# Illumina/canvas

Measured on AMD Instinct MI355X. Metric: genome-bins/sec (bin+clean+partition), higher is better.
Workload: dtype u8/int32 (bin), f32/f64 (clean, viterbi); 1 GPU; BASELINE configs[2]: whole-genome GRCh38 60x single sample, full bin+clean+partition HIP path on 1 MI355X per sample; bins_after_clean=4686240, bin_size=534, partition=PerSampleHMM, clean_flags=-g -s -r --local-sd-metric-file, segments=250, samples=1

## Files before the change

### canvas_amd/csrc/hmm.hip

```cpp
#include "common.hpp"
#include <type_traits>
#include "select.hpp"
#include "quantize.hpp"
#include <mutex>
#include <cmath>
#include <thread>
#include <cstring>
#include <limits>
#include <algorithm>

#define NSTATE 5

struct HmmParams {
    double logA[NSTATE][NSTATE];
    double logPi[NSTATE];
    int32_t tableLen;
    double maxThreshold;
};

__global__ void __launch_bounds__(256) k_keys_cov_f32(const double* __restrict__ cov, int64_t n, uint32_t* __restrict__ keys) {
    int64_t i = (int64_t)blockIdx.x * 256 + threadIdx.x;
    if (i < n) keys[i] = key_of_float((float)cov[i]);
}

// ... 232 lines not shown
            e = eNext;
        }
        __syncthreads();
        if (l < steps)
            psi[C.begin + t0 + l] = (uint16_t)(sPsi[0][l] | (sPsi[1][l] << 3) | (sPsi[2][l] << 6) | (sPsi[3][l] << 9) | (sPsi[4][l] << 12));
        __syncthreads();
    }
    double d[NSTATE];
#pragma unroll
    for (int i = 0; i < NSTATE; i++) d[i] = readlane_f64(delta, i);
    if (l == 0) {
        int best = -1; double m1 = NEG;
#pragma unroll
        for (int i = 0; i < NSTATE; i++) if (d[i] > m1) { best = i; m1 = d[i]; }
        lastState[cidx] = best;
    }
}


#define VB 128
#define VW0 16
#define VW 128
#define VW2 64
#define PQ 8
#define MAP_IDENT (0u | (1u << 3) | (2u << 6) | (3u << 9) | (4u << 12))
struct VitBlock { int32_t chrom; int32_t t0; };
struct __attribute__((aligned(4))) VecI4 { int v[4]; };
struct __attribute__((aligned(8))) VecD2 { double v[2]; };
struct __attribute__((aligned(2))) VecH8 { uint32_t w[4]; };

template <int J, bool TWO = false>
__device__ __forceinline__ void vit_state(const double (&d)[NSTATE], double e, const HmmParams& P, double& outDelta, uint32_t& outArg) {
    const double NEG = -1.7976931348623157e308;
    const double cOff = e + P.logA[J == 0 ? 1 : 0][J], cDiag = e + P.logA[J][J];
    const double t_0 = d[0] + (TWO ? (J == 0 ? cDiag : cOff) : (e + P.logA[0][J]));
    const double t_1 = d[1] + (TWO ? (J == 1 ? cDiag : cOff) : (e + P.logA[1][J]));
    const double t_2 = d[2] + (TWO ? (J == 2 ? cDiag : cOff) : (e + P.logA[2][J]));
    const double t_3 = d[3] + (TWO ? (J == 3 ? cDiag : cOff) : (e + P.logA[3][J]));
    const double t_4 = d[4] + (TWO ? (J == 4 ? cDiag : cOff) : (e + P.logA[4][J]));
    double a = __builtin_fmax(__builtin_fmax(__builtin_fmax(t_0, t_1), __builtin_fmax(t_2, t_3)), t_4);
    uint32_t ia = t_3 == a ? 3u : 4u;
    ia = t_2 == a ? 2u : ia; ia = t_1 == a ? 1u : ia; ia = t_0 == a ? 0u : ia;
    if (!(a > NEG)) { a = NEG; ia = 0; }
    outDelta = a; outArg = ia;
}
template <bool TWO = false>
__device__ __forceinline__ uint32_t vit_step5(double (&d)[NSTATE], const double (&e)[NSTATE], const HmmParams& P) {
    double n0, n1, n2, n3, n4; uint32_t a0, a1, a2, a3, a4;
    vit_state<0, TWO>(d, e[0], P, n0, a0); vit_state<1, TWO>(d, e[1], P, n1, a1); vit_state<2, TWO>(d, e[2], P, n2, a2);
    vit_state<3, TWO>(d, e[3], P, n3, a3); vit_state<4, TWO>(d, e[4], P, n4, a4);
    d[0] = n0; d[1] = n1; d[2] = n2; d[3] = n3; d[4] = n4;
    return a0 | (a1 << 3) | (a2 << 6) | (a3 << 9) | (a4 << 12);
}
__device__ __forceinline__ void vit_init5(double (&d)[NSTATE], const double (&e)[NSTATE], const HmmParams& P) {
#pragma unroll
    for (int j = 0; j < NSTATE; j++) { double lik = e[j] + P.logA[0][j]; d[j] = P.logPi[j] + lik - P.logA[0][j]; }
}
__device__ __forceinline__ int vit_best5(const double (&d)[NSTATE]) {
    int best = -1; double m1 = -1.7976931348623157e308;
#pragma unroll
    for (int i = 0; i < NSTATE; i++) if (d[i] > m1) { best = i; m1 = d[i]; }
    return best;
}
__device__ __forceinline__ uint32_t map_get(uint32_t m, uint32_t j) { return (m >> (3u * j)) & 7u; }
__device__ __forceinline__ uint32_t map_compose(uint32_t outer, uint32_t inner) {
    return map_get(outer, map_get(inner, 0)) | (map_get(outer, map_get(inner, 1)) << 3) | (map_get(outer, map_get(inner, 2)) << 6) |
           (map_get(outer, map_get(inner, 3)) << 9) | (map_get(outer, map_get(inner, 4)) << 12);
}
__device__ __forceinline__ double sel5(const double (&d)[NSTATE], uint32_t i) {
    double r = d[0];
    r = i == 1 ? d[1] : r; r = i == 2 ? d[2] : r; r = i == 3 ? d[3] : r; r = i == 4 ? d[4] : r;
    return r;
}
__device__ __forceinline__ void vit_emissions(double (&e)[NSTATE], const double* __restrict__ sTab, const double* __restrict__ logPmf, bool useLds, int tableLen, int k) {
    if (useLds) {
#pragma unroll
        for (int j = 0; j < NSTATE; j++) e[j] = sTab[k * NSTATE + j];
    } else {
#pragma unroll
        for (int j = 0; j < NSTATE; j++) e[j] = logPmf[(size_t)j * tableLen + k];
    }
}
__device__ __forceinline__ void vit_stage_table(double* sTab, const double* __restrict__ logPmf, int tableLen, bool useLds) {
    if (useLds) for (int i = threadIdx.x; i < tableLen * NSTATE; i += blockDim.x) { int s = i / tableLen, k = i - s * tableLen; sTab[k * NSTATE + s] = logPmf[i]; }
    __syncthreads();
}
__device__ __forceinline__ int wave_max_i32(int v) {
#pragma unroll
    for (int d = 32; d >= 1; d >>= 1) { int o = __shfl_xor(v, d); v = o > v ? o : v; }
    return v;
}

template <typename T> __device__ __forceinline__ void make_block_entry(const int32_t* __restrict__ first, int nchr, int i, int per, T* __restrict__ out) {
    int lo = 0, hi = nchr - 1;
    while (lo < hi) { int mid = (lo + hi + 1) >> 1; if (first[mid] <= i) lo = mid; else hi = mid - 1; }
    while (lo < nchr - 1 && first[lo + 1] <= i) lo++;
    T b; b.chrom = lo; b.t0 = (i - first[lo]) * per;
    out[i] = b;
}
template <typename T>
__global__ void __launch_bounds__(256) k_make_blocks(const int32_t* __restrict__ first, int nchr, int n, int per, T* __restrict__ out) {
    const int i = blockIdx.x * 256 + threadIdx.x;
    if (i < n) make_block_entry(first, nchr, i, per, out);
}

#define HMM_BYVAL 64
struct HmmDescPack { HmmChrom chroms[HMM_BYVAL]; int64_t off[HMM_BYVAL + 1]; int32_t first[HMM_BYVAL + 1], firstChunk[HMM_BYVAL + 1], firstS[HMM_BYVAL + 1], firstGroup[HMM_BYVAL + 1]; };
struct HmmDescDev { HmmChrom* chroms; int64_t* off; int32_t* first; int32_t* firstChunk; int32_t* firstS; int32_t* firstGroup; };
template <typename VB_T, typename BB_T>
__global__ void __launch_bounds__(256) k_hmm_setup(const HmmDescPack pack, int usePack, HmmDescDev D, int nchr,
                                                   int nblocks, int nblocksS, int nchunks, int vb, int vbs, int bbChunk, VB_T* __restrict__ vBlocks, VB_T* __restrict__ sBlocks, BB_T* __restrict__ bChunks,
                                                   const double* __restrict__ cov, int64_t N, double maxThreshold, int32_t* __restrict__ idx, int32_t* __restrict__ dLast, int32_t* __restrict__ dFail) {
    const int32_t* first = usePack ? pack.first : D.first; const int32_t* firstS = usePack ? pack.firstS : D.firstS; const int32_t* firstChunk = usePack ? pack.firstChunk : D.firstChunk;
    if (usePack && blockIdx.x == 0) {
        for (int c = threadIdx.x; c < nchr; c += 256) D.chroms[c] = pack.chroms[c];
        for (int c = threadIdx.x; c <= nchr; c += 256) { D.off[c] = pack.off[c]; D.first[c] = pack.first[c]; D.firstChunk[c] = pack.firstChunk[c]; D.firstS[c] = pack.firstS[c]; D.firstGroup[c] = pack.firstGroup[c]; }
    }
    const int64_t i = (int64_t)blockIdx.x * 256 + threadIdx.x;
    if (i < nblocks) make_block_entry(first, nchr, (int)i, vb, vBlocks);
    if (i < nblocksS) make_block_entry(firstS, nchr, (int)i, vbs, sBlocks);
    if (i < nchunks) make_block_entry(firstChunk, nchr, (int)i, bbChunk, bChunks);
    if (i < nchr) { dLast[i] = -1; dFail[i] = 0; }
    if (cov && i < N) {
        double x = cov[i];
        x = x > maxThreshold ? maxThreshold : x;
        const int32_t k = (int32_t)rint(x);
        idx[i] = k < 0 ? 0 : k;
    }
}

template <bool useLds, bool TWO>
__global__ void __launch_bounds__(64) k_vit_spec(const VitBlock* __restrict__ blocks, int nblocks, const HmmChrom* __restrict__ chroms, const int32_t* __restrict__ idx,
                                                 const double* __restrict__ logPmf, HmmParams P, uint16_t* __restrict__ psi, uint16_t* __restrict__ maps,
                                                 int32_t* __restrict__ lastGuess, int leadIn, const int32_t* __restrict__ todo, int vb) {
    extern __shared__ double sTab[];
    vit_stage_table(sTab, logPmf, P.tableLen, useLds);
    const int b = blockIdx.x * 64 + threadIdx.x;
    const bool actBlock = b < nblocks;
    const VitBlock B = blocks[actBlock ? b : nblocks - 1];
    const HmmChrom C = chroms[B.chrom];
    const int64_t tBeg = B.t0, tEnd = (B.t0 + vb < C.T) ? B.t0 + vb : C.T;
    const int64_t ts = tBeg > leadIn ? tBeg - leadIn : 0;
    const bool act = actBlock && (!todo || todo[B.chrom]);
// ... 43 lines not shown
    };
    const int leadMin = -wave_max_i32(nsteps > 0 ? -lead : -0x7FFFFFFF);
    int s0 = 1;
    for (; s0 + PQ <= leadMin && s0 < maxSteps; s0 += PQ) group(s0, std::false_type{});
    for (; s0 < maxSteps; s0 += PQ) group(s0, std::true_type{});
    if (act) {
        maps[b] = (uint16_t)fm;
        if (tEnd == C.T) lastGuess[B.chrom] = vit_best5(d);
    }
}

#define CHR_LDS_CAP 1024
__device__ __forceinline__ const int64_t* stage_chr_offsets(const int64_t* __restrict__ chrOff, int nchr, int64_t* sOff) {
    if (nchr + 1 > CHR_LDS_CAP) return chrOff;
    for (int k = threadIdx.x; k <= nchr; k += blockDim.x) sOff[k] = chrOff[k];
    __syncthreads();
    return sOff;
}
__device__ __forceinline__ int chrom_of_bin(const int64_t* off, int nchr, int64_t g) {
    int lo = 0, hi = nchr - 1;
    while (lo < hi) { const int mid = (lo + hi + 1) >> 1; if (off[mid] <= g) lo = mid; else hi = mid - 1; }
    return lo;
}
#define VBS (VB / 2)
__global__ void __launch_bounds__(256) k_pair_maps(const VitBlock* __restrict__ blocks, int nblocks, const HmmChrom* __restrict__ chroms, const int32_t* __restrict__ firstS,
                                                   const uint16_t* __restrict__ mapsS, uint16_t* __restrict__ maps, const int32_t* __restrict__ todo) {
    const int b = blockIdx.x * 256 + threadIdx.x;
    if (b >= nblocks) return;
    const VitBlock B = blocks[b];
    if (todo && !todo[B.chrom]) return;
    const int64_t T = chroms[B.chrom].T;
    const int s0 = firstS[B.chrom] + B.t0 / VBS;
    uint32_t m = mapsS[s0];
#pragma unroll
    for (int k = 1; k < VB / VBS; k++) if (B.t0 + (int64_t)k * VBS < T) m = map_compose(m, mapsS[s0 + k]);
    maps[b] = (uint16_t)m;
}

__global__ void __launch_bounds__(256) k_vit_increments(const HmmChrom* __restrict__ chroms, int nchr, const int64_t* __restrict__ chrOff, const int32_t* __restrict__ idx,
                                                        const double* __restrict__ logPmf, HmmParams P, const int32_t* __restrict__ state, int64_t N, double* __restrict__ D) {
    __shared__ int64_t sOff[CHR_LDS_CAP];
    const int64_t* off = stage_chr_offsets(chrOff, nchr, sOff);
    int64_t g = (int64_t)blockIdx.x * 256 + threadIdx.x;
    if (g >= N) return;
    const int s1 = state[g], sPrev = state[g > 0 ? g - 1 : 0], ix = idx[g];
    const int lo = chrom_of_bin(off, nchr, g);
    const int64_t begin = chroms[lo].begin;
// ... 390 lines not shown
    for (int j = 0; j < NSTATE; j++) {
        const uint32_t p = map_get(pk, j);
        const double dp = pick5(p, S.d[0], S.d[1], S.d[2], S.d[3], S.d[4]);
        const bool vp = ((S.valid >> p) & 1u) != 0;
        const double step = e[j] + la5[j];
        const bool isCur = j == sCur, fromPrev = (int)p == S.sPrev;
        const double viaPrev = S.Dprev + step, viaAnc = dp + step;
        const double r0 = vp ? viaAnc : S.d[j], r1 = fromPrev ? viaPrev : r0, r = isCur ? Dt : r1;
        nd[j] = r; nv |= (isCur || fromPrev || vp) ? (1u << j) : 0u;
    }
#pragma unroll
    for (int j = 0; j < NSTATE; j++) S.d[j] = on ? nd[j] : S.d[j];
    S.valid = on ? nv : S.valid; S.Dprev = on ? Dt : S.Dprev; S.sPrev = on ? sCur : S.sPrev;
}
template <bool useLds>
__device__ __forceinline__ void ver_block_step(VerState& S, const HmmParams& P, const double* __restrict__ sTab, const double* __restrict__ logPmf, bool on, int k, int sCur,
                                               double v, uint32_t pk) {
    double e[NSTATE], dn[NSTATE];
    vit_emissions(e, sTab, logPmf, useLds, P.tableLen, on ? k : 0);
    const double Dt = S.Dprev + v;
#pragma unroll
    for (int j = 0; j < NSTATE; j++) dn[j] = S.d[j];
    const uint32_t got = vit_step5(dn, e, P);
    S.bad = S.bad || (on && (S.valid != 31u || got != pk || sel5(dn, (uint32_t)(on ? sCur : 0)) != Dt));
    S.why |= on ? ((S.valid != 31u ? 2u : 0u) | (got != pk ? 4u : 0u) | (sel5(dn, (uint32_t)(on ? sCur : 0)) != Dt ? 8u : 0u)) : 0u;
#pragma unroll
    for (int j = 0; j < NSTATE; j++) S.d[j] = on ? dn[j] : S.d[j];
    S.Dprev = on ? Dt : S.Dprev; S.sPrev = on ? sCur : S.sPrev;
}
template <bool useLds, bool LEAD>
__device__ __forceinline__ void ver_phase(VerState& S, const LogA25& A, const HmmParams& P, const double* __restrict__ sTab, const double* __restrict__ logPmf,
                                          const int32_t* __restrict__ ixp, const int32_t* __restrict__ stp, const double* __restrict__ vp, const uint16_t* __restrict__ ppp, int cnt) {
    const int maxCnt = wave_max_i32(cnt);
    int kq[PQ], sq[PQ]; double vq[PQ]; uint32_t pq[PQ];
#pragma unroll
    for (int u = 0; u < PQ; u++) { const bool in = u < cnt; kq[u] = in ? ixp[u] : 0; sq[u] = in ? stp[u] : 0; vq[u] = in ? vp[u] : 0.0; pq[u] = in ? ppp[u] : 0u; }
    for (int j0 = 0; j0 < maxCnt; j0 += PQ) {
        int kn[PQ], sn[PQ]; double vn[PQ]; VecH8 pn;
        if (j0 + 2 * PQ <= cnt) {
            const int o = j0 + PQ;
            const VecI4 ka = *reinterpret_cast<const VecI4*>(ixp + o), kb = *reinterpret_cast<const VecI4*>(ixp + o + 4);
            const VecI4 sa = *reinterpret_cast<const VecI4*>(stp + o), sb = *reinterpret_cast<const VecI4*>(stp + o + 4);
            const VecD2 v0 = *reinterpret_cast<const VecD2*>(vp + o), v1 = *reinterpret_cast<const VecD2*>(vp + o + 2), v2 = *reinterpret_cast<const VecD2*>(vp + o + 4),
                        v3 = *reinterpret_cast<const VecD2*>(vp + o + 6);
            pn = *reinterpret_cast<const VecH8*>(ppp + o);
#pragma unroll
            for (int u = 0; u < 4; u++) { kn[u] = ka.v[u]; kn[4 + u] = kb.v[u]; sn[u] = sa.v[u]; sn[4 + u] = sb.v[u]; }
            vn[0] = v0.v[0]; vn[1] = v0.v[1]; vn[2] = v1.v[0]; vn[3] = v1.v[1]; vn[4] = v2.v[0]; vn[5] = v2.v[1]; vn[6] = v3.v[0]; vn[7] = v3.v[1];
        } else {
#pragma unroll
            for (int u = 0; u < PQ; u++) { const bool in = j0 + PQ + u < cnt; kn[u] = in ? ixp[j0 + PQ + u] : 0; sn[u] = in ? stp[j0 + PQ + u] : 0; vn[u] = in ? vp[j0 + PQ + u] : 0.0; }
#pragma unroll
            for (int u = 0; u < 4; u++) pn.w[u] = (uint32_t)(j0 + PQ + 2 * u < cnt ? ppp[j0 + PQ + 2 * u] : (uint16_t)0) | ((uint32_t)(j0 + PQ + 2 * u + 1 < cnt ? ppp[j0 + PQ + 2 * u + 1] : (uint16_t)0) << 16);
        }
#pragma unroll
        for (int u = 0; u < PQ; u++) {
            if (LEAD) ver_lead_step<useLds>(S, A, sTab, logPmf, P.tableLen, j0 + u < cnt, kq[u], sq[u], vq[u], pq[u]);
            else ver_block_step<useLds>(S, P, sTab, logPmf, j0 + u < cnt, kq[u], sq[u], vq[u], pq[u]);
        }
        __builtin_amdgcn_sched_barrier(0);
#pragma unroll
        for (int u = 0; u < PQ; u++) { kq[u] = kn[u]; sq[u] = sn[u]; vq[u] = vn[u]; pq[u] = (pn.w[u >> 1] >> (16 * (u & 1))) & 0xFFFFu; }
    }
}
template <bool useLds>
__global__ void __launch_bounds__(64) k_vit_verify(const VitBlock* __restrict__ blocks, int nblocks, const HmmChrom* __restrict__ chroms, const int32_t* __restrict__ idx,
                                                   const double* __restrict__ logPmf, HmmParams P, const uint16_t* __restrict__ psi,
                                                   const int32_t* __restrict__ state, const double* __restrict__ V, const double* __restrict__ carry, const int32_t* __restrict__ lastGuess,
                                                   int32_t* __restrict__ fail, int leadIn, const int32_t* __restrict__ todo) {
    extern __shared__ double sTab[];
    vit_stage_table(sTab, logPmf, P.tableLen, useLds);
    const int b = blockIdx.x * 64 + threadIdx.x;
    const bool actBlock = b < nblocks;
    const VitBlock B = blocks[actBlock ? b : nblocks - 1];
    const HmmChrom C = chroms[B.chrom];
    const int64_t tBeg = B.t0, tEnd = (B.t0 + VB < C.T) ? B.t0 + VB : C.T;
    const int64_t ts = tBeg > leadIn ? tBeg - leadIn : 0;
    const bool act = actBlock && (!todo || todo[B.chrom]);
    const int nsteps = act ? (int)(tEnd - ts) : 0;
    const int maxSteps = wave_max_i32(nsteps);
    const int32_t* __restrict__ ix = idx + C.begin + ts;
    const int32_t* __restrict__ st = state + C.begin + ts;
    const double* __restrict__ Vc = V + C.begin + ts;
    const uint16_t* __restrict__ pp = psi + C.begin + ts;
    VerState S;
#pragma unroll
    for (int j = 0; j < NSTATE; j++) S.d[j] = 0.0;
    S.valid = 0; S.bad = false; S.why = 0;
    S.Dprev = carry[C.begin + ts];
    S.sPrev = ts > 0 ? state[C.begin + ts - 1] : -1;
    LogA25 A;
#define LOGA_LOAD(i, j) A.a##i##j = P.logA[i][j]; asm volatile("" : "+v"(A.a##i##j));
    LOGA_LOAD(0, 0) LOGA_LOAD(0, 1) LOGA_LOAD(0, 2) LOGA_LOAD(0, 3) LOGA_LOAD(0, 4) LOGA_LOAD(1, 0) LOGA_LOAD(1, 1) LOGA_LOAD(1, 2) LOGA_LOAD(1, 3) LOGA_LOAD(1, 4)
    LOGA_LOAD(2, 0) LOGA_LOAD(2, 1) LOGA_LOAD(2, 2) LOGA_LOAD(2, 3) LOGA_LOAD(2, 4) LOGA_LOAD(3, 0) LOGA_LOAD(3, 1) LOGA_LOAD(3, 2) LOGA_LOAD(3, 3) LOGA_LOAD(3, 4)
    LOGA_LOAD(4, 0) LOGA_LOAD(4, 1) LOGA_LOAD(4, 2) LOGA_LOAD(4, 3) LOGA_LOAD(4, 4)
#undef LOGA_LOAD
    const int lead = (int)(tBeg - ts);
    if (nsteps > 0) {
        if (ts == 0) {
            double e[NSTATE];
            vit_emissions(e, sTab, logPmf, useLds, P.tableLen, ix[0]);
            const double Dt = S.Dprev + Vc[0];
            const int sCur = st[0];
            vit_init5(S.d, e, P); S.valid = 31u;
            if (sel5(S.d, (uint32_t)sCur) != Dt) { S.bad = true; S.why |= 16u; }
            S.Dprev = Dt; S.sPrev = sCur;
        } else ver_lead_step<useLds>(S, A, sTab, logPmf, P.tableLen, true, ix[0], st[0], Vc[0], (uint32_t)pp[0]);
    }
    const int start2 = lead > 1 ? lead : 1;
    ver_phase<useLds, true>(S, A, P, sTab, logPmf, ix + 1, st + 1, Vc + 1, pp + 1, nsteps > 0 && lead > 1 ? lead - 1 : 0);
    ver_phase<useLds, false>(S, A, P, sTab, logPmf, ix + start2, st + start2, Vc + start2, pp + start2, nsteps > start2 ? nsteps - start2 : 0);
    double (&d)[NSTATE] = S.d; const uint32_t valid = S.valid; bool bad = S.bad;
    uint32_t why = S.why;
    if (act && tEnd == C.T) { if (valid != 31u || vit_best5(d) != lastGuess[B.chrom]) { bad = true; why |= 32u; } }
    if (act && bad) atomicOr(&fail[B.chrom], (int32_t)(1u | why));
}

__global__ void k_vit_corrupt(uint16_t* __restrict__ psi, int64_t at, int j) {
    if (threadIdx.x == 0 && blockIdx.x == 0) { const uint32_t sh = 3u * (uint32_t)j; uint32_t v = psi[at], p = (v >> sh) & 7u; psi[at] = (uint16_t)((v & ~(7u << sh)) | (((p + 1u) % 5u) << sh)); }
}

__global__ void __launch_bounds__(256) k_bt_maps(const VitBlock* __restrict__ blocks, int nblocks, const HmmChrom* __restrict__ chroms, const uint16_t* __restrict__ psi,
                                                 uint16_t* __restrict__ maps) {
    int b = blockIdx.x * 256 + threadIdx.x;
    if (b >= nblocks) return;
    const VitBlock B = blocks[b];
    const HmmChrom C = chroms[B.chrom];
    const int64_t tBeg = B.t0 > 0 ? B.t0 : 1, tEnd = (B.t0 + VB < C.T) ? B.t0 + VB : C.T;
// ... 300 lines not shown
        else { idx[cnt++] = mm; idx[cnt++] = mm + mid; }
    } else {
        idx[cnt++] = mid;
        if ((n - 1) % 4 == 0) { int64_t k = (n - 1) / 4; idx[cnt++] = k - 1; idx[cnt++] = k; idx[cnt++] = 3 * k; idx[cnt++] = 3 * k + 1; }
        else { int64_t k = (n - 3) / 4; idx[cnt++] = k; idx[cnt++] = k + 1; idx[cnt++] = 3 * k + 1; idx[cnt++] = 3 * k + 2; }
    }
}
static void quartile_val(int64_t n, const float* v, float& q1, float& q2, float& q3) {
    int64_t mid = n / 2;
    if (n % 2 == 0) {
        q2 = (v[0] + v[1]) / 2;
        if (mid % 2 == 0) { q1 = (v[2] + v[3]) / 2; q3 = (v[4] + v[5]) / 2; } else { q1 = v[2]; q3 = v[3]; }
    } else {
        q2 = v[0];
        if ((n - 1) % 4 == 0) { q1 = (v[1] * 0.25f) + (v[2] * 0.75f); q3 = (v[3] * 0.75f) + (v[4] * 0.25f); }
        else { q1 = (v[1] * 0.75f) + (v[2] * 0.25f); q3 = (v[3] * 0.25f) + (v[4] * 0.75f); }
    }
}

static inline unsigned nblk2(int64_t n, int per) { return (unsigned)((n + per - 1) / per); }

struct HmmLists {
    std::vector<HmmChrom> chroms;
    std::vector<int32_t> firstBlock, firstGroup, firstS, firstChunk;
    int nblocks = 0, ngroups = 0, nblocksS = 0, nchunks = 0;
};
static HmmLists hmm_lists(int32_t nchr, const int64_t* h_chr_offset) {
    HmmLists L;
    L.chroms.resize(nchr); L.firstBlock.resize(nchr + 1);
    for (int c = 0; c < nchr; c++) {
        L.chroms[c].begin = h_chr_offset[c]; L.chroms[c].T = h_chr_offset[c + 1] - h_chr_offset[c];
        L.firstBlock[c] = L.nblocks;
        if (L.chroms[c].T > 10) L.nblocks += (int)((L.chroms[c].T + VB - 1) / VB);
    }
    L.firstBlock[nchr] = L.nblocks;
    L.firstGroup.resize(nchr + 1);
    for (int c = 0; c < nchr; c++) { L.firstGroup[c] = L.ngroups; L.ngroups += (L.firstBlock[c + 1] - L.firstBlock[c] + 63) / 64; }
    L.firstGroup[nchr] = L.ngroups;
    L.firstS.resize(nchr + 1);
    for (int c = 0; c < nchr; c++) { L.firstS[c] = L.nblocksS; if (L.chroms[c].T > 10) L.nblocksS += (int)((L.chroms[c].T + VBS - 1) / VBS); }
    L.firstS[nchr] = L.nblocksS;
    L.firstChunk.resize(nchr + 1);
    for (int c = 0; c < nchr; c++) {
        L.firstChunk[c] = L.nchunks;
        if (L.chroms[c].T > 10) L.nchunks += (int)((L.chroms[c].T + BB_CHUNK - 1) / BB_CHUNK);
    }
    L.firstChunk[nchr] = L.nchunks;
    return L;
}

enum { BB_MODE_CHAIN = 0, BB_MODE_SCAN = 1, BB_MODE_PIECES = 2 };
struct BbWork { double* chunkSum; double* chunkBase; BbChunkOut* chunkOut; BbCross* cross; ParFn* at64Fn; uint8_t* at64Rank; unsigned long long* chunkBits; BbPost* post; };
static void bb_work_size(WsSizer& sz, int nchunks) {
    sz.take<double>(nchunks + 1); sz.take<double>(nchunks + 1); sz.take<BbChunkOut>(nchunks + 1);
    sz.take<BbCross>((size_t)nchunks * BB_MAXC + 1); sz.take<ParFn>((size_t)nchunks * 16 + 1); sz.take<uint8_t>((size_t)nchunks * 16 + 8);
    sz.take<unsigned long long>(nchunks + 1); sz.take<BbPost>((size_t)nchunks * BB_MAXC + 1);
}
static BbWork bb_work_carve(WsCarver& ws, int nchunks) {
    BbWork W;
    W.chunkSum = ws.take<double>(nchunks + 1); W.chunkBase = ws.take<double>(nchunks + 1); W.chunkOut = ws.take<BbChunkOut>(nchunks + 1);
    W.cross = ws.take<BbCross>((size_t)nchunks * BB_MAXC + 1); W.at64Fn = ws.take<ParFn>((size_t)nchunks * 16 + 1); W.at64Rank = ws.take<uint8_t>((size_t)nchunks * 16 + 8);
    W.chunkBits = ws.take<unsigned long long>(nchunks + 1); W.post = ws.take<BbPost>((size_t)nchunks * BB_MAXC + 1);
    return W;
}
// ... 31 lines not shown
        p = end + 1;
    }
    if (nf != 3 && nf != 4) CANVAS_FAIL(ctx, CANVAS_ERR_INVALID, "CANVAS_HMM_TEST_CORRUPT: 1, c:t:j or c:t:j:k");
    if (v[0] >= nchr) CANVAS_FAIL(ctx, CANVAS_ERR_INVALID, "CANVAS_HMM_TEST_CORRUPT: no such chromosome");
    const int64_t T = h_chr_offset[v[0] + 1] - h_chr_offset[v[0]];
    if (T <= 10 || v[1] < 1 || v[1] >= T) CANVAS_FAIL(ctx, CANVAS_ERR_INVALID, "CANVAS_HMM_TEST_CORRUPT: the step must be 1 .. T-1 of a chromosome of more than ten bins");
    if (v[2] >= NSTATE) CANVAS_FAIL(ctx, CANVAS_ERR_INVALID, "CANVAS_HMM_TEST_CORRUPT: the state must be 0 .. 4");
    if (nf == 4 && (v[3] < 1 || v[3] > 5)) CANVAS_FAIL(ctx, CANVAS_ERR_INVALID, "CANVAS_HMM_TEST_CORRUPT: 1 .. 5 corrupted attempts");
    K.chrom = (int)v[0]; K.t = v[1]; K.state = (int)v[2]; K.attempts = nf == 4 ? (int)v[3] : 1; K.retry = nf == 4;
    return CANVAS_OK;
}

struct HmmEmis { int32_t* idx = nullptr; double* dTab = nullptr;
                 const double* indexCov = nullptr; };
struct SegPost { const int32_t* d_start; const int32_t* d_stop; int32_t maxDist; int32_t* d_segment_id; int64_t nseg = 0; bool valid = false; };
static void enqueue_segment_ids(canvas_ctx* ctx, const int64_t* dOff, int nchr, const int32_t* d_state, const int32_t* d_start, const int32_t* d_stop, int64_t N, int32_t maxDist,
                                uint8_t* flags, uint32_t* blockCnt, unsigned long long* dTot, int32_t* d_segment_id, unsigned* totSeq = nullptr, unsigned seq = 0);
template <class PrepareA, class PrepareB>
static int32_t hmm_pipeline(canvas_ctx* ctx, int32_t nchr, const int64_t* h_chr_offset, size_t extraBytes, PrepareA prepareA, PrepareB prepareB, int32_t* d_state, SegPost* seg = nullptr,
                            bool descByValue = false ) {
    const int64_t N = h_chr_offset[nchr];
    VitCorrupt corrupt;
    { int32_t rcc = vit_corrupt_parse(ctx, nchr, h_chr_offset, corrupt); if (rcc) return rcc; }
    const HmmLists L = hmm_lists(nchr, h_chr_offset);
    const std::vector<HmmChrom>& chroms = L.chroms;
    const std::vector<int32_t>&firstBlock = L.firstBlock, &firstGroup = L.firstGroup, &firstS = L.firstS, &firstChunk = L.firstChunk;
    const int nblocks = L.nblocks, ngroups = L.ngroups, nblocksS = L.nblocksS, nchunks = L.nchunks;
    const int nbSeg = (int)nblk2(N, 2048);
    WsSizer sz;
    sz.take<BbChunk>(nchunks + 1); sz.take<int32_t>(nchr + 1); bb_work_size(sz, nchunks);
    sz.take<uint16_t>(N + 8); sz.take<HmmChrom>(nchr); sz.take<int32_t>(nchr);
    sz.take<int32_t>(nchr + 1); sz.take<uint16_t>(nblocks + 8); sz.take<int8_t>(nblocks + 8);
    sz.take<int64_t>(nchr + 1); sz.take<VitBlock>(nblocks + 1); sz.take<double>(N); sz.take<double>(N + 64); sz.take<int32_t>(nchr); sz.take<int32_t>(nchr);
    sz.take<VitBlock>(nblocksS + 1); sz.take<uint16_t>(nblocksS + 8); sz.take<int32_t>(nchr + 1);
    sz.take<int32_t>(nchr + 1); sz.take<uint16_t>(nblocks + 8); sz.take<uint16_t>(ngroups + 8); sz.take<int8_t>(ngroups + 8);
    sz.take<char>(8 * 256 + (size_t)nchr * 64 + 64);
    if (seg) { sz.take<uint8_t>(N + 16); sz.take<uint32_t>(nbSeg + 1); sz.take<unsigned long long>(1); }
    int32_t rc = canvas_ws_reserve(ctx, sz.off + extraBytes + 65536); if (rc) return rc;
    rc = canvas_pin_reserve(ctx, (size_t)nchr * 4 + 64); if (rc) return rc;
    WsCarver ws(ctx->ws);
    uint16_t* psi = ws.take<uint16_t>(N + 8);
    HmmChrom* dChroms = ws.take<HmmChrom>(nchr); int32_t* dLast = ws.take<int32_t>(nchr);
    int32_t* dFirst = ws.take<int32_t>(nchr + 1);
    uint16_t* dMaps = ws.take<uint16_t>(nblocks + 8); (void)ws.take<int8_t>(nblocks + 8);
    int64_t* dOffDev = ws.take<int64_t>(nchr + 1);
    VitBlock* dVBlocks = ws.take<VitBlock>(nblocks + 1); double* dD = ws.take<double>(N); double* dCarry = ws.take<double>(N + 64); int32_t* dFail = ws.take<int32_t>(nchr); int32_t* dRedo = ws.take<int32_t>(nchr);
    int32_t* dFirstGroup = ws.take<int32_t>(nchr + 1); uint16_t* dPre = ws.take<uint16_t>(nblocks + 8); uint16_t* dGmap = ws.take<uint16_t>(ngroups + 8);
    int8_t* dGentry = ws.take<int8_t>(ngroups + 8);
    VitBlock* dSBlocks = ws.take<VitBlock>(nblocksS + 1); uint16_t* dMapsS = ws.take<uint16_t>(nblocksS + 8); int32_t* dFirstS = ws.take<int32_t>(nchr + 1);
    BbChunk* dBChunks = ws.take<BbChunk>(nchunks + 1); int32_t* dFirstChunk = ws.take<int32_t>(nchr + 1);
    const BbWork bbWork = bb_work_carve(ws, nchunks);
    uint8_t* segFlags = nullptr; uint32_t* segBlockCnt = nullptr; unsigned long long* segTot = nullptr;
    if (seg) { segFlags = ws.take<uint8_t>(N + 16); segBlockCnt = ws.take<uint32_t>(nbSeg + 1); segTot = ws.take<unsigned long long>(1); seg->valid = false; }

    const bool byVal = descByValue && nchr <= HMM_BYVAL;
    HmmDescPack pack;
    {
        auto al = [](size_t v) { return (v + 255) & ~size_t(255); };
        const size_t oCh = 0, oFirst = al((size_t)nchr * sizeof(HmmChrom)), oOff = oFirst + al((size_t)(nchr + 1) * 4), oChunk = oOff + al((size_t)(nchr + 1) * 8),
                     oS = oChunk + al((size_t)(nchr + 1) * 4), oG = oS + al((size_t)(nchr + 1) * 4), total = oG + al((size_t)(nchr + 1) * 4);
        char* dBlob = ws.take<char>(total);
        if (byVal) {
            memset(&pack, 0, sizeof pack);
            memcpy(pack.chroms, chroms.data(), (size_t)nchr * sizeof(HmmChrom)); memcpy(pack.off, h_chr_offset, (size_t)(nchr + 1) * 8); memcpy(pack.first, firstBlock.data(), (size_t)(nchr + 1) * 4);
            memcpy(pack.firstChunk, firstChunk.data(), (size_t)(nchr + 1) * 4); memcpy(pack.firstS, firstS.data(), (size_t)(nchr + 1) * 4); memcpy(pack.firstGroup, firstGroup.data(), (size_t)(nchr + 1) * 4);
        } else {
            std::vector<char> blob(total, 0);
            memcpy(blob.data() + oCh, chroms.data(), (size_t)nchr * sizeof(HmmChrom)); memcpy(blob.data() + oFirst, firstBlock.data(), (size_t)(nchr + 1) * 4);
            memcpy(blob.data() + oOff, h_chr_offset, (size_t)(nchr + 1) * 8); memcpy(blob.data() + oChunk, firstChunk.data(), (size_t)(nchr + 1) * 4);
            memcpy(blob.data() + oS, firstS.data(), (size_t)(nchr + 1) * 4); memcpy(blob.data() + oG, firstGroup.data(), (size_t)(nchr + 1) * 4);
            rc = canvas_h2d_small(ctx, dBlob, blob.data(), total); if (rc) return rc;
        }
        dChroms = (HmmChrom*)(dBlob + oCh); dFirst = (int32_t*)(dBlob + oFirst); dOffDev = (int64_t*)(dBlob + oOff); dFirstChunk = (int32_t*)(dBlob + oChunk);
        dFirstS = (int32_t*)(dBlob + oS); dFirstGroup = (int32_t*)(dBlob + oG);
    }
    HmmParams P; HmmEmis E;
    ctx->hmm_dispersion = 1e9;
    rc = prepareA(ws, P, E, (const HmmChrom*)dChroms, (const int64_t*)dOffDev); if (rc) return rc;
    {
        const int64_t most = std::max<int64_t>(std::max<int64_t>(E.indexCov ? N : 0, nblocks), std::max<int64_t>(std::max(nblocksS, nchunks), nchr));
        HmmDescDev DD{dChroms, dOffDev, dFirst, dFirstChunk, dFirstS, dFirstGroup};
        hipLaunchKernelGGL((k_hmm_setup<VitBlock, BbChunk>), dim3(nblk2(most, 256)), dim3(256), 0, ctx->stream, pack, byVal ? 1 : 0, DD, nchr, nblocks, nblocksS, nchunks, VB, VBS, BB_CHUNK,
                           dVBlocks, dSBlocks, dBChunks, E.indexCov, N, P.maxThreshold, E.idx, dLast, dFail);
    }
    rc = prepareB(ws, P, E); if (rc) return rc;
    int32_t* idx = E.idx; double* dTab = E.dTab;
    size_t tabBytes = (size_t)NSTATE * P.tableLen * 8;
    size_t lds = tabBytes <= 48 * 1024 ? tabBytes : 0;
    for (int c = 0; c < nchr; c++)
        if (chroms[c].T <= 10 && chroms[c].T > 0)
            hipLaunchKernelGGL(k_fill_i32, dim3(nblk2(chroms[c].T, 256)), dim3(256), 0, ctx->stream, d_state, chroms[c].begin, chroms[c].begin + chroms[c].T, -1);
    const unsigned laneGrid = (unsigned)((nblocks + 63) / 64);
    auto backtrack = [&](bool haveMaps) {
        if (nblocks > 0) {
            if (!haveMaps) hipLaunchKernelGGL(k_bt_maps, dim3(nblk2(nblocks, 256)), dim3(256), 0, ctx->stream, dVBlocks, nblocks, dChroms, psi, dMaps);
            hipLaunchKernelGGL(k_bt_group, dim3(ngroups), dim3(64), 0, ctx->stream, dFirst, dFirstGroup, nchr, dMaps, dPre, dGmap);
            hipLaunchKernelGGL(k_bt_gchain, dim3(nchr), dim3(64), 0, ctx->stream, dFirstGroup, dLast, dGmap, dGentry);
            hipLaunchKernelGGL(k_bt_states, dim3(nblk2(nblocks, 4)), dim3(256), 0, ctx->stream, dVBlocks, nblocks, dChroms, psi, dFirst, dFirstGroup, dPre, dGentry, d_state);
        }
    };
    bool twoValuedAll = true;
    for (int i = 0; i < NSTATE; i++) for (int j = 0; j < NSTATE; j++) {
        const double ref = i == j ? P.logA[0][0] : P.logA[0][1];
        if (memcmp(&P.logA[i][j], &ref, sizeof(double)) != 0) twoValuedAll = false;
    }
    const bool speculative = cvx_hook("CANVAS_HMM_SEQUENTIAL") == nullptr;
    std::vector<int32_t> redo;
    int32_t* hFail = (int32_t*)ctx->pin; unsigned long long* hSegTot = (unsigned long long*)((char*)ctx->pin + (((size_t)nchr * 4 + 15) & ~size_t(15)));
    bool segEnqueued = false; unsigned* hSegSeq = (unsigned*)(hSegTot + 1); unsigned segSeq = 0;
    if (speculative && nblocks > 0) {
        ProfScope ps(ctx, "viterbi");
        const int32_t* dTodo = nullptr;
        ctx->hmm_retry = 0;
        const int vwEnv = cvx_hook("CANVAS_HMM_LEAD") ? atoi(cvx_hook("CANVAS_HMM_LEAD")) : 0;
        const int vw0 = vwEnv > 0 ? vwEnv : (ctx->hmm_dispersion < 0.20 ? VW0 : (ctx->hmm_dispersion < 0.30 ? 64 : VW));
        const int nAttempts = 5;
        for (int attempt = 0; attempt < nAttempts; attempt++) {
            const int mult = attempt <= 1 ? 1 : (attempt == 2 ? 8 : (attempt == 3 ? 64 : 512));
            const int leadSpec = attempt == 0 ? vw0 : mult * VW, leadVer = mult * VW2;
            cvx_prof_count(ctx, "viterbi_attempt");
            if (attempt > 0) CANVAS_HIP_TRY(ctx, hipMemsetAsync(dFail, 0, nchr * 4, ctx->stream));
            const dim3 gs((unsigned)((nblocksS + 63) / 64));
            const bool twoValued = twoValuedAll && attempt < 3;
            if (lds && twoValued) hipLaunchKernelGGL((k_vit_spec<true, true>), gs, dim3(64), lds, ctx->stream, dSBlocks, nblocksS, dChroms, idx, dTab, P, psi, dMapsS, dLast, leadSpec, dTodo, VBS);
            else if (lds) hipLaunchKernelGGL((k_vit_spec<true, false>), gs, dim3(64), lds, ctx->stream, dSBlocks, nblocksS, dChroms, idx, dTab, P, psi, dMapsS, dLast, leadSpec, dTodo, VBS);
            else if (twoValued) hipLaunchKernelGGL((k_vit_spec<false, true>), gs, dim3(64), 0, ctx->stream, dSBlocks, nblocksS, dChroms, idx, dTab, P, psi, dMapsS, dLast, leadSpec, dTodo, VBS);
            else hipLaunchKernelGGL((k_vit_spec<false, false>), gs, dim3(64), 0, ctx->stream, dSBlocks, nblocksS, dChroms, idx, dTab, P, psi, dMapsS, dLast, leadSpec, dTodo, VBS);
            hipLaunchKernelGGL(k_pair_maps, dim3(nblk2(nblocks, 256)), dim3(256), 0, ctx->stream, dVBlocks, nblocks, dChroms, dFirstS, dMapsS, dMaps, dTodo);
            if (attempt < corrupt.attempts) hipLaunchKernelGGL(k_vit_corrupt, dim3(1), dim3(64), 0, ctx->stream, psi, chroms[corrupt.chrom].begin + corrupt.t, corrupt.state);
            backtrack(true);
            hipLaunchKernelGGL(k_vit_increments, dim3(nblk2(N, 256)), dim3(256), 0, ctx->stream, dChroms, nchr, dOffDev, idx, dTab, P, d_state, N, dD);
            const char* bbMode = cvx_hook("CANVAS_HMM_BACKBONE");
            const int bb = ((bbMode && !strcmp(bbMode, "chain")) || (attempt > 1 && !bbMode)) ? BB_MODE_CHAIN : ((bbMode && !strcmp(bbMode, "scan")) ? BB_MODE_SCAN : BB_MODE_PIECES);
            enqueue_backbone(ctx, bb, nchr, nchunks, dChroms, dBChunks, dFirstChunk, dD, dCarry, dFail, dTodo, bbWork);
            if (lds) hipLaunchKernelGGL((k_vit_verify<true>), dim3(laneGrid), dim3(64), lds, ctx->stream, dVBlocks, nblocks, dChroms, idx, dTab, P, psi, d_state, dD, dCarry, dLast, dFail, leadVer, dTodo);
            else hipLaunchKernelGGL((k_vit_verify<false>), dim3(laneGrid), dim3(64), 0, ctx->stream, dVBlocks, nblocks, dChroms, idx, dTab, P, psi, d_state, dD, dCarry, dLast, dFail, leadVer, dTodo);
            CANVAS_HIP_TRY(ctx, hipMemcpyAsync(hFail, dFail, nchr * 4, hipMemcpyDeviceToHost, ctx->stream));
            if (seg && attempt == 0 && (!corrupt.on || corrupt.retry)) {
                (void)segTot;
                segSeq = cvx_mail_arm(ctx, hSegSeq);
                enqueue_segment_ids(ctx, dOffDev, nchr, d_state, seg->d_start, seg->d_stop, N, seg->maxDist, segFlags, segBlockCnt, hSegTot , seg->d_segment_id, hSegSeq, segSeq);
                segEnqueued = true;
            }
            CANVAS_HIP_TRY(ctx, hipStreamSynchronize(ctx->stream));
            redo.clear();
            for (int c = 0; c < nchr; c++) if (hFail[c] && chroms[c].T > 10) redo.push_back(c);
            if (!redo.empty() && cvx_hook("CANVAS_HMM_DEBUG_FAIL")) { fprintf(stderr, "viterbi attempt %d (lead-in x%d):", attempt, mult); for (int c : redo) fprintf(stderr, " chr%d(T=%lld, why=0x%x)", c, (long long)chroms[c].T, (unsigned)hFail[c]); fprintf(stderr, "\n"); }
            if (redo.empty() || (corrupt.on && !corrupt.retry) || cvx_hook("CANVAS_HMM_NO_RETRY")) break;
            if (attempt < nAttempts - 1) {
                if (attempt == 0) { ctx->hmm_retry = (int)redo.size(); { ProfScope pr(ctx, "viterbi_retry"); } }
                int32_t rcq = canvas_h2d_small(ctx, dRedo, hFail, nchr * 4); if (rcq) return rcq;
                dTodo = dRedo;
            }
        }
        if (seg && segEnqueued && redo.empty() && ctx->hmm_retry == 0) { int32_t rcm = cvx_mail_await(ctx, hSegSeq, segSeq, "PerSampleHMM: segment count"); if (rcm) return rcm; seg->valid = true; seg->nseg = (int64_t)*hSegTot; }
    } else {
        for (int c = 0; c < nchr; c++) redo.push_back(c);
    }
    if (!redo.empty()) {
// ... 385 lines not shown
```

Before: 2.015 billion bins/s.

## Retile Viterbi verify into smaller blocks with shorter first-attempt lead-in

On the first attempt the verify pass now uses its own block list of length VC=96 instead of VB=128, and a shorter lead-in (16) when dispersion is low. The speculative block size is halved (VB/4). The carry lookup is aligned down to a multiple of 64 and the remaining prefix is summed from V, which adds per-thread work. The dCur comparison is rewritten branch-light with pick5. The aim is more parallel verify lanes and less sequential lead-in work, at the cost of more blocks, more map composition and possibly more retries if the shorter lead-in fails to converge.

```diff
diff --git a/canvas_amd/csrc/hmm.hip b/canvas_amd/csrc/hmm.hip
--- a/canvas_amd/csrc/hmm.hip
+++ b/canvas_amd/csrc/hmm.hip
@@ -278,6 +278,8 @@
 #define VW0 16
 #define VW 128
 #define VW2 64
+#define VW2S 16
+#define VC 96
 #define PQ 8
 #define MAP_IDENT (0u | (1u << 3) | (2u << 6) | (3u << 9) | (4u << 12))
 struct VitBlock { int32_t chrom; int32_t t0; };
@@ -323,11 +325,6 @@
     return map_get(outer, map_get(inner, 0)) | (map_get(outer, map_get(inner, 1)) << 3) | (map_get(outer, map_get(inner, 2)) << 6) |
            (map_get(outer, map_get(inner, 3)) << 9) | (map_get(outer, map_get(inner, 4)) << 12);
 }
-__device__ __forceinline__ double sel5(const double (&d)[NSTATE], uint32_t i) {
-    double r = d[0];
-    r = i == 1 ? d[1] : r; r = i == 2 ? d[2] : r; r = i == 3 ? d[3] : r; r = i == 4 ? d[4] : r;
-    return r;
-}
 __device__ __forceinline__ void vit_emissions(double (&e)[NSTATE], const double* __restrict__ sTab, const double* __restrict__ logPmf, bool useLds, int tableLen, int k) {
     if (useLds) {
 #pragma unroll
@@ -361,20 +358,22 @@
 }
 
 #define HMM_BYVAL 64
-struct HmmDescPack { HmmChrom chroms[HMM_BYVAL]; int64_t off[HMM_BYVAL + 1]; int32_t first[HMM_BYVAL + 1], firstChunk[HMM_BYVAL + 1], firstS[HMM_BYVAL + 1], firstGroup[HMM_BYVAL + 1]; };
-struct HmmDescDev { HmmChrom* chroms; int64_t* off; int32_t* first; int32_t* firstChunk; int32_t* firstS; int32_t* firstGroup; };
+struct HmmDescPack { HmmChrom chroms[HMM_BYVAL]; int64_t off[HMM_BYVAL + 1]; int32_t first[HMM_BYVAL + 1], firstChunk[HMM_BYVAL + 1], firstS[HMM_BYVAL + 1], firstGroup[HMM_BYVAL + 1], firstC[HMM_BYVAL + 1]; };
+struct HmmDescDev { HmmChrom* chroms; int64_t* off; int32_t* first; int32_t* firstChunk; int32_t* firstS; int32_t* firstGroup; int32_t* firstC; };
 template <typename VB_T, typename BB_T>
 __global__ void __launch_bounds__(256) k_hmm_setup(const HmmDescPack pack, int usePack, HmmDescDev D, int nchr,
-                                                   int nblocks, int nblocksS, int nchunks, int vb, int vbs, int bbChunk, VB_T* __restrict__ vBlocks, VB_T* __restrict__ sBlocks, BB_T* __restrict__ bChunks,
+                                                   int nblocks, int nblocksS, int nblocksC, int nchunks, int vb, int vbs, int vc, int bbChunk, VB_T* __restrict__ vBlocks, VB_T* __restrict__ sBlocks, VB_T* __restrict__ cBlocks, BB_T* __restrict__ bChunks,
                                                    const double* __restrict__ cov, int64_t N, double maxThreshold, int32_t* __restrict__ idx, int32_t* __restrict__ dLast, int32_t* __restrict__ dFail) {
     const int32_t* first = usePack ? pack.first : D.first; const int32_t* firstS = usePack ? pack.firstS : D.firstS; const int32_t* firstChunk = usePack ? pack.firstChunk : D.firstChunk;
+    const int32_t* firstC = usePack ? pack.firstC : D.firstC;
     if (usePack && blockIdx.x == 0) {
         for (int c = threadIdx.x; c < nchr; c += 256) D.chroms[c] = pack.chroms[c];
-        for (int c = threadIdx.x; c <= nchr; c += 256) { D.off[c] = pack.off[c]; D.first[c] = pack.first[c]; D.firstChunk[c] = pack.firstChunk[c]; D.firstS[c] = pack.firstS[c]; D.firstGroup[c] = pack.firstGroup[c]; }
+        for (int c = threadIdx.x; c <= nchr; c += 256) { D.off[c] = pack.off[c]; D.first[c] = pack.first[c]; D.firstChunk[c] = pack.firstChunk[c]; D.firstS[c] = pack.firstS[c]; D.firstGroup[c] = pack.firstGroup[c]; D.firstC[c] = pack.firstC[c]; }
     }
     const int64_t i = (int64_t)blockIdx.x * 256 + threadIdx.x;
     if (i < nblocks) make_block_entry(first, nchr, (int)i, vb, vBlocks);
     if (i < nblocksS) make_block_entry(firstS, nchr, (int)i, vbs, sBlocks);
+    if (i < nblocksC) make_block_entry(firstC, nchr, (int)i, vc, cBlocks);
     if (i < nchunks) make_block_entry(firstChunk, nchr, (int)i, bbChunk, bChunks);
     if (i < nchr) { dLast[i] = -1; dFail[i] = 0; }
     if (cov && i < N) {
@@ -464,7 +463,7 @@
     while (lo < hi) { const int mid = (lo + hi + 1) >> 1; if (off[mid] <= g) lo = mid; else hi = mid - 1; }
     return lo;
 }
-#define VBS (VB / 2)
+#define VBS (VB / 4)
 __global__ void __launch_bounds__(256) k_pair_maps(const VitBlock* __restrict__ blocks, int nblocks, const HmmChrom* __restrict__ chroms, const int32_t* __restrict__ firstS,
                                                    const uint16_t* __restrict__ mapsS, uint16_t* __restrict__ maps, const int32_t* __restrict__ todo) {
     const int b = blockIdx.x * 256 + threadIdx.x;
@@ -901,8 +900,13 @@
 #pragma unroll
     for (int j = 0; j < NSTATE; j++) dn[j] = S.d[j];
     const uint32_t got = vit_step5(dn, e, P);
-    S.bad = S.bad || (on && (S.valid != 31u || got != pk || sel5(dn, (uint32_t)(on ? sCur : 0)) != Dt));
-    S.why |= on ? ((S.valid != 31u ? 2u : 0u) | (got != pk ? 4u : 0u) | (sel5(dn, (uint32_t)(on ? sCur : 0)) != Dt ? 8u : 0u)) : 0u;
+    double n0 = dn[0], n1 = dn[1], n2 = dn[2], n3 = dn[3], n4 = dn[4];
+    asm volatile("" : "+v"(n0), "+v"(n1), "+v"(n2), "+v"(n3), "+v"(n4));
+    const double dCur = pick5((uint32_t)sCur, n0, n1, n2, n3, n4);
+    const uint32_t why = (S.valid != 31u ? 2u : 0u) | (got != pk ? 4u : 0u) | (dCur != Dt ? 8u : 0u);
+    S.bad = S.bad | (on & (why != 0u));
+    S.why |= on ? why : 0u;
+    dn[0] = n0; dn[1] = n1; dn[2] = n2; dn[3] = n3; dn[4] = n4;
 #pragma unroll
     for (int j = 0; j < NSTATE; j++) S.d[j] = on ? dn[j] : S.d[j];
     S.Dprev = on ? Dt : S.Dprev; S.sPrev = on ? sCur : S.sPrev;
@@ -946,15 +950,16 @@
 __global__ void __launch_bounds__(64) k_vit_verify(const VitBlock* __restrict__ blocks, int nblocks, const HmmChrom* __restrict__ chroms, const int32_t* __restrict__ idx,
                                                    const double* __restrict__ logPmf, HmmParams P, const uint16_t* __restrict__ psi,
                                                    const int32_t* __restrict__ state, const double* __restrict__ V, const double* __restrict__ carry, const int32_t* __restrict__ lastGuess,
-                                                   int32_t* __restrict__ fail, int leadIn, const int32_t* __restrict__ todo) {
+                                                   int32_t* __restrict__ fail, int leadIn, const int32_t* __restrict__ todo, int vc) {
     extern __shared__ double sTab[];
     vit_stage_table(sTab, logPmf, P.tableLen, useLds);
     const int b = blockIdx.x * 64 + threadIdx.x;
     const bool actBlock = b < nblocks;
     const VitBlock B = blocks[actBlock ? b : nblocks - 1];
     const HmmChrom C = chroms[B.chrom];
-    const int64_t tBeg = B.t0, tEnd = (B.t0 + VB < C.T) ? B.t0 + VB : C.T;
+    const int64_t tBeg = B.t0, tEnd = (B.t0 + vc < C.T) ? B.t0 + vc : C.T;
     const int64_t ts = tBeg > leadIn ? tBeg - leadIn : 0;
+    const int64_t tc = ts & ~(int64_t)63;
     const bool act = actBlock && (!todo || todo[B.chrom]);
     const int nsteps = act ? (int)(tEnd - ts) : 0;
     const int maxSteps = wave_max_i32(nsteps);
@@ -966,7 +971,18 @@
 #pragma unroll
     for (int j = 0; j < NSTATE; j++) S.d[j] = 0.0;
     S.valid = 0; S.bad = false; S.why = 0;
-    S.Dprev = carry[C.begin + ts];
+    S.Dprev = carry[C.begin + tc];
+    {
+        const int pre = act ? (int)(ts - tc) : 0, maxPre = wave_max_i32(pre);
+        const double* __restrict__ Vp = V + C.begin + tc;
+        for (int i0 = 0; i0 < maxPre; i0 += 16) {
+            double r[16];
+#pragma unroll
+            for (int u = 0; u < 16; u++) r[u] = i0 + u < pre ? Vp[i0 + u] : 0.0;
+#pragma unroll
+            for (int u = 0; u < 16; u++) S.Dprev = i0 + u < pre ? S.Dprev + r[u] : S.Dprev;
+        }
+    }
     S.sPrev = ts > 0 ? state[C.begin + ts - 1] : -1;
     LogA25 A;
 #define LOGA_LOAD(i, j) A.a##i##j = P.logA[i][j]; asm volatile("" : "+v"(A.a##i##j));
@@ -982,7 +998,7 @@
             const double Dt = S.Dprev + Vc[0];
             const int sCur = st[0];
             vit_init5(S.d, e, P); S.valid = 31u;
-            if (sel5(S.d, (uint32_t)sCur) != Dt) { S.bad = true; S.why |= 16u; }
+            if (pick5((uint32_t)sCur, S.d[0], S.d[1], S.d[2], S.d[3], S.d[4]) != Dt) { S.bad = true; S.why |= 16u; }
             S.Dprev = Dt; S.sPrev = sCur;
         } else ver_lead_step<useLds>(S, A, sTab, logPmf, P.tableLen, true, ix[0], st[0], Vc[0], (uint32_t)pp[0]);
     }
@@ -1329,10 +1345,10 @@
 
 struct HmmLists {
     std::vector<HmmChrom> chroms;
-    std::vector<int32_t> firstBlock, firstGroup, firstS, firstChunk;
-    int nblocks = 0, ngroups = 0, nblocksS = 0, nchunks = 0;
+    std::vector<int32_t> firstBlock, firstGroup, firstS, firstC, firstChunk;
+    int nblocks = 0, ngroups = 0, nblocksS = 0, nblocksC = 0, nchunks = 0;
 };
-static HmmLists hmm_lists(int32_t nchr, const int64_t* h_chr_offset) {
+static HmmLists hmm_lists(int32_t nchr, const int64_t* h_chr_offset, int vc = VB) {
     HmmLists L;
     L.chroms.resize(nchr); L.firstBlock.resize(nchr + 1);
     for (int c = 0; c < nchr; c++) {
@@ -1347,6 +1363,9 @@
     L.firstS.resize(nchr + 1);
     for (int c = 0; c < nchr; c++) { L.firstS[c] = L.nblocksS; if (L.chroms[c].T > 10) L.nblocksS += (int)((L.chroms[c].T + VBS - 1) / VBS); }
     L.firstS[nchr] = L.nblocksS;
+    L.firstC.resize(nchr + 1);
+    for (int c = 0; c < nchr; c++) { L.firstC[c] = L.nblocksC; if (L.chroms[c].T > 10) L.nblocksC += (int)((L.chroms[c].T + vc - 1) / vc); }
+    L.firstC[nchr] = L.nblocksC;
     L.firstChunk.resize(nchr + 1);
     for (int c = 0; c < nchr; c++) {
         L.firstChunk[c] = L.nchunks;
@@ -1424,17 +1443,18 @@
     const int64_t N = h_chr_offset[nchr];
     VitCorrupt corrupt;
     { int32_t rcc = vit_corrupt_parse(ctx, nchr, h_chr_offset, corrupt); if (rcc) return rcc; }
-    const HmmLists L = hmm_lists(nchr, h_chr_offset);
+    const int vc = VC;
+    const HmmLists L = hmm_lists(nchr, h_chr_offset, vc);
     const std::vector<HmmChrom>& chroms = L.chroms;
-    const std::vector<int32_t>&firstBlock = L.firstBlock, &firstGroup = L.firstGroup, &firstS = L.firstS, &firstChunk = L.firstChunk;
-    const int nblocks = L.nblocks, ngroups = L.ngroups, nblocksS = L.nblocksS, nchunks = L.nchunks;
+    const std::vector<int32_t>&firstBlock = L.firstBlock, &firstGroup = L.firstGroup, &firstS = L.firstS, &firstC = L.firstC, &firstChunk = L.firstChunk;
+    const int nblocks = L.nblocks, ngroups = L.ngroups, nblocksS = L.nblocksS, nblocksC = L.nblocksC, nchunks = L.nchunks;
     const int nbSeg = (int)nblk2(N, 2048);
     WsSizer sz;
     sz.take<BbChunk>(nchunks + 1); sz.take<int32_t>(nchr + 1); bb_work_size(sz, nchunks);
     sz.take<uint16_t>(N + 8); sz.take<HmmChrom>(nchr); sz.take<int32_t>(nchr);
     sz.take<int32_t>(nchr + 1); sz.take<uint16_t>(nblocks + 8); sz.take<int8_t>(nblocks + 8);
     sz.take<int64_t>(nchr + 1); sz.take<VitBlock>(nblocks + 1); sz.take<double>(N); sz.take<double>(N + 64); sz.take<int32_t>(nchr); sz.take<int32_t>(nchr);
-    sz.take<VitBlock>(nblocksS + 1); sz.take<uint16_t>(nblocksS + 8); sz.take<int32_t>(nchr + 1);
+    sz.take<VitBlock>(nblocksS + 1); sz.take<uint16_t>(nblocksS + 8); sz.take<int32_t>(nchr + 1); sz.take<VitBlock>(nblocksC + 1);
     sz.take<int32_t>(nchr + 1); sz.take<uint16_t>(nblocks + 8); sz.take<uint16_t>(ngroups + 8); sz.take<int8_t>(ngroups + 8);
     sz.take<char>(8 * 256 + (size_t)nchr * 64 + 64);
     if (seg) { sz.take<uint8_t>(N + 16); sz.take<uint32_t>(nbSeg + 1); sz.take<unsigned long long>(1); }
@@ -1450,40 +1470,43 @@
     int32_t* dFirstGroup = ws.take<int32_t>(nchr + 1); uint16_t* dPre = ws.take<uint16_t>(nblocks + 8); uint16_t* dGmap = ws.take<uint16_t>(ngroups + 8);
     int8_t* dGentry = ws.take<int8_t>(ngroups + 8);
     VitBlock* dSBlocks = ws.take<VitBlock>(nblocksS + 1); uint16_t* dMapsS = ws.take<uint16_t>(nblocksS + 8); int32_t* dFirstS = ws.take<int32_t>(nchr + 1);
+    VitBlock* dCBlocks = ws.take<VitBlock>(nblocksC + 1);
     BbChunk* dBChunks = ws.take<BbChunk>(nchunks + 1); int32_t* dFirstChunk = ws.take<int32_t>(nchr + 1);
     const BbWork bbWork = bb_work_carve(ws, nchunks);
     uint8_t* segFlags = nullptr; uint32_t* segBlockCnt = nullptr; unsigned long long* segTot = nullptr;
     if (seg) { segFlags = ws.take<uint8_t>(N + 16); segBlockCnt = ws.take<uint32_t>(nbSeg + 1); segTot = ws.take<unsigned long long>(1); seg->valid = false; }
 
     const bool byVal = descByValue && nchr <= HMM_BYVAL;
-    HmmDescPack pack;
+    HmmDescPack pack; int32_t* dFirstC = nullptr;
     {
         auto al = [](size_t v) { return (v + 255) & ~size_t(255); };
         const size_t oCh = 0, oFirst = al((size_t)nchr * sizeof(HmmChrom)), oOff = oFirst + al((size_t)(nchr + 1) * 4), oChunk = oOff + al((size_t)(nchr + 1) * 8),
-                     oS = oChunk + al((size_t)(nchr + 1) * 4), oG = oS + al((size_t)(nchr + 1) * 4), total = oG + al((size_t)(nchr + 1) * 4);
+                     oS = oChunk + al((size_t)(nchr + 1) * 4), oG = oS + al((size_t)(nchr + 1) * 4), oC = oG + al((size_t)(nchr + 1) * 4), total = oC + al((size_t)(nchr + 1) * 4);
         char* dBlob = ws.take<char>(total);
         if (byVal) {
             memset(&pack, 0, sizeof pack);
             memcpy(pack.chroms, chroms.data(), (size_t)nchr * sizeof(HmmChrom)); memcpy(pack.off, h_chr_offset, (size_t)(nchr + 1) * 8); memcpy(pack.first, firstBlock.data(), (size_t)(nchr + 1) * 4);
             memcpy(pack.firstChunk, firstChunk.data(), (size_t)(nchr + 1) * 4); memcpy(pack.firstS, firstS.data(), (size_t)(nchr + 1) * 4); memcpy(pack.firstGroup, firstGroup.data(), (size_t)(nchr + 1) * 4);
+            memcpy(pack.firstC, firstC.data(), (size_t)(nchr + 1) * 4);
         } else {
             std::vector<char> blob(total, 0);
             memcpy(blob.data() + oCh, chroms.data(), (size_t)nchr * sizeof(HmmChrom)); memcpy(blob.data() + oFirst, firstBlock.data(), (size_t)(nchr + 1) * 4);
             memcpy(blob.data() + oOff, h_chr_offset, (size_t)(nchr + 1) * 8); memcpy(blob.data() + oChunk, firstChunk.data(), (size_t)(nchr + 1) * 4);
             memcpy(blob.data() + oS, firstS.data(), (size_t)(nchr + 1) * 4); memcpy(blob.data() + oG, firstGroup.data(), (size_t)(nchr + 1) * 4);
+            memcpy(blob.data() + oC, firstC.data(), (size_t)(nchr + 1) * 4);
             rc = canvas_h2d_small(ctx, dBlob, blob.data(), total); if (rc) return rc;
         }
         dChroms = (HmmChrom*)(dBlob + oCh); dFirst = (int32_t*)(dBlob + oFirst); dOffDev = (int64_t*)(dBlob + oOff); dFirstChunk = (int32_t*)(dBlob + oChunk);
-        dFirstS = (int32_t*)(dBlob + oS); dFirstGroup = (int32_t*)(dBlob + oG);
+        dFirstS = (int32_t*)(dBlob + oS); dFirstGroup = (int32_t*)(dBlob + oG); dFirstC = (int32_t*)(dBlob + oC);
     }
     HmmParams P; HmmEmis E;
     ctx->hmm_dispersion = 1e9;
     rc = prepareA(ws, P, E, (const HmmChrom*)dChroms, (const int64_t*)dOffDev); if (rc) return rc;
     {
-        const int64_t most = std::max<int64_t>(std::max<int64_t>(E.indexCov ? N : 0, nblocks), std::max<int64_t>(std::max(nblocksS, nchunks), nchr));
-        HmmDescDev DD{dChroms, dOffDev, dFirst, dFirstChunk, dFirstS, dFirstGroup};
-        hipLaunchKernelGGL((k_hmm_setup<VitBlock, BbChunk>), dim3(nblk2(most, 256)), dim3(256), 0, ctx->stream, pack, byVal ? 1 : 0, DD, nchr, nblocks, nblocksS, nchunks, VB, VBS, BB_CHUNK,
-                           dVBlocks, dSBlocks, dBChunks, E.indexCov, N, P.maxThreshold, E.idx, dLast, dFail);
+        const int64_t most = std::max<int64_t>(std::max<int64_t>(E.indexCov ? N : 0, nblocks), std::max<int64_t>(std::max(std::max(nblocksS, nblocksC), nchunks), nchr));
+        HmmDescDev DD{dChroms, dOffDev, dFirst, dFirstChunk, dFirstS, dFirstGroup, dFirstC};
+        hipLaunchKernelGGL((k_hmm_setup<VitBlock, BbChunk>), dim3(nblk2(most, 256)), dim3(256), 0, ctx->stream, pack, byVal ? 1 : 0, DD, nchr, nblocks, nblocksS, nblocksC, nchunks, VB, VBS, vc, BB_CHUNK,
+                           dVBlocks, dSBlocks, dCBlocks, dBChunks, E.indexCov, N, P.maxThreshold, E.idx, dLast, dFail);
     }
     rc = prepareB(ws, P, E); if (rc) return rc;
     int32_t* idx = E.idx; double* dTab = E.dTab;
@@ -1492,7 +1515,6 @@
     for (int c = 0; c < nchr; c++)
         if (chroms[c].T <= 10 && chroms[c].T > 0)
             hipLaunchKernelGGL(k_fill_i32, dim3(nblk2(chroms[c].T, 256)), dim3(256), 0, ctx->stream, d_state, chroms[c].begin, chroms[c].begin + chroms[c].T, -1);
-    const unsigned laneGrid = (unsigned)((nblocks + 63) / 64);
     auto backtrack = [&](bool haveMaps) {
         if (nblocks > 0) {
             if (!haveMaps) hipLaunchKernelGGL(k_bt_maps, dim3(nblk2(nblocks, 256)), dim3(256), 0, ctx->stream, dVBlocks, nblocks, dChroms, psi, dMaps);
@@ -1516,10 +1538,14 @@
         ctx->hmm_retry = 0;
         const int vwEnv = cvx_hook("CANVAS_HMM_LEAD") ? atoi(cvx_hook("CANVAS_HMM_LEAD")) : 0;
         const int vw0 = vwEnv > 0 ? vwEnv : (ctx->hmm_dispersion < 0.20 ? VW0 : (ctx->hmm_dispersion < 0.30 ? 64 : VW));
+        const int vlEnv = cvx_hook("CANVAS_HMM_VERIFY_LEAD") ? atoi(cvx_hook("CANVAS_HMM_VERIFY_LEAD")) : 0;
+        const int vl0 = vlEnv > 0 ? vlEnv : (ctx->hmm_dispersion < 0.20 ? VW2S : VW2);
         const int nAttempts = 5;
         for (int attempt = 0; attempt < nAttempts; attempt++) {
             const int mult = attempt <= 1 ? 1 : (attempt == 2 ? 8 : (attempt == 3 ? 64 : 512));
-            const int leadSpec = attempt == 0 ? vw0 : mult * VW, leadVer = mult * VW2;
+            const int leadSpec = attempt == 0 ? vw0 : mult * VW, leadVer = attempt == 0 ? vl0 : mult * VW2;
+            const VitBlock* verBlocks = attempt == 0 ? dCBlocks : dVBlocks;
+            const int nVer = attempt == 0 ? nblocksC : nblocks, verLen = attempt == 0 ? vc : VB;
             cvx_prof_count(ctx, "viterbi_attempt");
             if (attempt > 0) CANVAS_HIP_TRY(ctx, hipMemsetAsync(dFail, 0, nchr * 4, ctx->stream));
             const dim3 gs((unsigned)((nblocksS + 63) / 64));
@@ -1535,8 +1561,9 @@
             const char* bbMode = cvx_hook("CANVAS_HMM_BACKBONE");
             const int bb = ((bbMode && !strcmp(bbMode, "chain")) || (attempt > 1 && !bbMode)) ? BB_MODE_CHAIN : ((bbMode && !strcmp(bbMode, "scan")) ? BB_MODE_SCAN : BB_MODE_PIECES);
             enqueue_backbone(ctx, bb, nchr, nchunks, dChroms, dBChunks, dFirstChunk, dD, dCarry, dFail, dTodo, bbWork);
-            if (lds) hipLaunchKernelGGL((k_vit_verify<true>), dim3(laneGrid), dim3(64), lds, ctx->stream, dVBlocks, nblocks, dChroms, idx, dTab, P, psi, d_state, dD, dCarry, dLast, dFail, leadVer, dTodo);
-            else hipLaunchKernelGGL((k_vit_verify<false>), dim3(laneGrid), dim3(64), 0, ctx->stream, dVBlocks, nblocks, dChroms, idx, dTab, P, psi, d_state, dD, dCarry, dLast, dFail, leadVer, dTodo);
+            const dim3 gv((unsigned)((nVer + 63) / 64));
+            if (lds) hipLaunchKernelGGL((k_vit_verify<true>), gv, dim3(64), lds, ctx->stream, verBlocks, nVer, dChroms, idx, dTab, P, psi, d_state, dD, dCarry, dLast, dFail, leadVer, dTodo, verLen);
+            else hipLaunchKernelGGL((k_vit_verify<false>), gv, dim3(64), 0, ctx->stream, verBlocks, nVer, dChroms, idx, dTab, P, psi, d_state, dD, dCarry, dLast, dFail, leadVer, dTodo, verLen);
             CANVAS_HIP_TRY(ctx, hipMemcpyAsync(hFail, dFail, nchr * 4, hipMemcpyDeviceToHost, ctx->stream));
             if (seg && attempt == 0 && (!corrupt.on || corrupt.retry)) {
                 (void)segTot;
```

Result: faster. 2.096 billion bins/s (median of 6 runs) (+4.0%).
